# RozDavid/UnScene3D

Hardware: AMD Instinct MI355X
Metric: training scenes/sec (Res16UNet34C+Mask3D, 150k voxels) (higher is better)
Workload: dtype f32

## Files before the change

include/usc3d.h:

```cpp
#ifndef USC3D_H
#define USC3D_H

#include <stdint.h>

#ifdef __cplusplus
extern "C" {
#endif

typedef void* usc_stream_t;

enum usc_status {
  USC_OK = 0,
  USC_ERR_ARG = -1,
  USC_ERR_LAUNCH = -2,
  USC_ERR_RANGE = -3
};

const char* usc_last_error(void);
int usc_abi_version(void);
const char* usc_build_info(void);
int usc_device_count(void);


int usc_voxel_floor_f64(const double* xyz, int64_t n, double voxel_size,
// ... 65 lines not shown
                     usc_stream_t s);

int64_t usc_spconv_gather_gemm_ws_bytes(int64_t n_out, int32_t cin,
                                        int32_t cout, int32_t K);
int usc_spconv_gather_gemm(const float* in, int64_t n_in, int32_t cin,
                           const float* W, int32_t K, int32_t cout,
                           const int32_t* nbr, int64_t n_out,
                           const float* bias, float* out, int32_t accumulate, int32_t w_transposed,
                           void* ws, int64_t ws_bytes, usc_stream_t s);

int usc_spconv_pairs_gemm(const float* in, int32_t cin, const float* W,
                          int32_t K, int32_t cout, const int32_t* rows_in,
                          const int32_t* rows_out, const int64_t* koff,
                          int64_t P_capacity, float* out, usc_stream_t s);

int usc_cast_bf16(const float* in, int64_t n, uint16_t* out, usc_stream_t s);
int usc_spconv_pack_w_bf16(const float* W, int32_t K, int32_t cin, int32_t cout,
                           uint16_t* Wp, usc_stream_t s);
int64_t usc_spconv_gather_gemm_bf16_ws_bytes(int64_t n_out, int32_t cin,
                                             int32_t cout, int32_t K);
int usc_spconv_gather_gemm_bf16(const uint16_t* in, int64_t n_in, int32_t cin,
                                const uint16_t* Wp, int32_t K, int32_t cout,
                                const int32_t* nbr, int64_t n_out,
                                const float* bias, float* out, int32_t accumulate,
                                void* ws, int64_t ws_bytes, usc_stream_t s);

int64_t usc_spconv_wgrad_ws_bytes(int32_t K, int32_t cin, int32_t cout);
int usc_spconv_wgrad(const float* a, int32_t cin, const float* b, int32_t cout,
                     int32_t K, const int32_t* a_idx, const int32_t* b_idx,
                     const int64_t* koff, int64_t n_rows, float* dW, int32_t accumulate, void* ws,
                     int64_t ws_bytes, usc_stream_t s);
int64_t usc_spconv_wgrad_ws_bytes_rows(int32_t K, int32_t cin, int32_t cout,
                                       int64_t n_rows);
int64_t usc_spconv_wgrad_table_ws_bytes(int32_t K, int32_t cin, int32_t cout);
int usc_spconv_wgrad_table(const float* in, int32_t cin, const float* dy, int32_t cout, const int32_t* nbr, int32_t K,
                           int64_t n_out, float* dW, int32_t accumulate, void* ws, int64_t ws_bytes, usc_stream_t s);

void usc_spconv_wgrad_grid_limit(int32_t max_workgroups);
int32_t usc_spconv_wgrad_group_max(void);
int usc_spconv_wgrad_group_ok(int32_t R, int32_t cin, int32_t cout, int32_t K, int64_t n_rows);
int usc_spconv_wgrad_group(int32_t R, const float* const* a, const float* const* b, float* const* dW, int32_t cin,
                           int32_t cout, int32_t K, const int32_t* a_idx, const int32_t* b_idx, const int64_t* koff,
                           int64_t n_rows, int32_t accumulate, usc_stream_t s);

typedef struct usc_kmap {
  const int32_t* nbr;
  const int32_t* perm;
  const uint32_t* tile_mask;
  const int32_t* pair_in;
  const int32_t* pair_out;
  const int64_t* koff;
  int64_t n_in, n_out;
  int64_t pair_capacity;
  int32_t K;
  int32_t reserved;
} usc_kmap;

enum usc_conv_kind { USC_CONV_SAME = 0, USC_CONV_DOWN = 1, USC_CONV_UP = 2 };

typedef struct usc_bn {
  const float* gamma;
  const float* beta;
  float* running_mean;
  float* running_var;
  int64_t* num_batches_tracked;
  float eps, momentum;
// ... 398 lines not shown
```

unscene3d_amd/_lib.py:

```python
from __future__ import annotations

import ctypes as C
import os

import torch

_HERE = os.path.dirname(os.path.abspath(__file__))
LIB_PATH = os.environ.get("USC3D_LIB") or os.path.join(_HERE, "libusc3d_hip.so")

_p = C.c_void_p
_i32 = C.c_int32
_i64 = C.c_int64
_f64 = C.c_double
_f32 = C.c_float

class KMap(C.Structure):
    _fields_ = [("nbr", _p), ("perm", _p), ("tile_mask", _p), ("pair_in", _p), ("pair_out", _p), ("koff", _p),
                ("n_in", _i64), ("n_out", _i64), ("pair_capacity", _i64), ("K", _i32), ("reserved", _i32)]


class BNDesc(C.Structure):
    _fields_ = [("gamma", _p), ("beta", _p), ("running_mean", _p), ("running_var", _p), ("num_batches_tracked", _p),
                ("eps", _f32), ("momentum", _f32), ("c", _i32), ("training", _i32)]

# ... 26 lines not shown
    "usc_coordmap_capacity": (_i64, [_i64]),
    "usc_coordmap_ws_bytes": (_i64, [_i64]),
    "usc_coordmap_build": (C.c_int, [_p, _i64, _i32, _p, _p, _i64, _p, _p, _p, _p, _p, _i64, _p]),
    "usc_morton_cell_ids": (C.c_int, [_p, _i64, _i32, _i32, _i32, _i32, _i32, _p, _p]),
    "usc_kernel_map_cube": (C.c_int, [_p, _i64, _i32, _i32, _p, _p, _i64, _p, _p]),
    "usc_kernel_map_down2": (C.c_int, [_p, _i64, _i32, _p, _p, _i64, _p, _p, _p]),
    "usc_rulebook_ws_bytes": (_i64, [_i64, _i64]),
    "usc_rulebook_compact": (C.c_int, [_p, _i64, _i64, _p, _p, _p, _p, _i64, _p]),
    "usc_weight_transpose": (C.c_int, [_p, _i32, _i32, _i32, _i32, _p, _p]),
    "usc_spconv_plan": (C.c_int, [_i32, _i64, _i32, _i32, _i32]),
    "usc_spconv_gather_gemm_ws_bytes": (_i64, [_i64, _i32, _i32, _i32]),
    "usc_spconv_gather_gemm": (C.c_int, [_p, _i64, _i32, _p, _i32, _i32, _p, _i64, _p, _p, _i32, _i32, _p, _i64, _p]),
    "usc_rowsort_ws_bytes": (_i64, [_i32, _i64]),
    "usc_rowsort_build": (C.c_int, [_p, _i32, _i64, _p, _p, _p, _i64, _p]),
    "usc_spconv_sorted_ws_bytes": (_i64, [_i64, _i32, _i32, _i32]),
    "usc_spconv_sorted_gemm": (C.c_int, [_p, _i64, _i32, _p, _i32, _i32, _p, _p, _p, _i64, _p, _p, _i32, _i32, _p, _i64, _p]),
    "usc_spconv_sorted_gemm_ex": (C.c_int, [_p, _i64, _i32, _p, _i32, _i32, _p, _p, _p, _i64, _p, _p, _i32, _i32, _p, _i64, _p, _p]),
    "usc_group_reduce": (C.c_int, [_p, _i32, _i64, _i32, _p, _i32, _p, _p]),
    "usc_bn_tile_max_rows": (C.c_int64, []),
    "usc_bn_tile_ok": (C.c_int, [_i64, _i32]),
    "usc_bn_tile_ws_bytes": (C.c_int64, [_i32]),
    "usc_bn_tile_forward": (C.c_int, [_p, _i32, _p, _i64, _i32, _p, _p, _f32, _f32, _p, _p, _p, _p, _p, _p, _p, _p, _i32, _p,
                                      _p, _i64, _p]),
    "usc_bn_tile_backward": (C.c_int, [_p, _i32, _i32, _p, _p, _p, _p, _p, _p, _i64, _i32, _i32, _i32, _p, _p, _p, _p, _p,
                                       _i64, _p]),
    "usc_spconv_pairs_gemm": (C.c_int, [_p, _i32, _p, _i32, _i32, _p, _p, _p, _i64, _p, _p]),
    "usc_cast_bf16": (C.c_int, [_p, _i64, _p, _p]),
    "usc_spconv_pack_w_bf16": (C.c_int, [_p, _i32, _i32, _i32, _p, _p]),
    "usc_spconv_gather_gemm_bf16_ws_bytes": (_i64, [_i64, _i32, _i32, _i32]),
    "usc_spconv_gather_gemm_bf16": (C.c_int, [_p, _i64, _i32, _p, _i32, _i32, _p, _i64, _p, _p, _i32, _p, _i64, _p]),
    "usc_spconv_wgrad_ws_bytes": (_i64, [_i32, _i32, _i32]),
    "usc_spconv_wgrad": (C.c_int, [_p, _i32, _p, _i32, _i32, _p, _p, _p, _i64, _p, _i32, _p, _i64, _p]),
    "usc_spconv_wgrad_ws_bytes_rows": (_i64, [_i32, _i32, _i32, _i64]),
    "usc_step_size": (_i32, []),
    "usc_program_ws_bytes": (_i64, [_sp, _i32]),
    "usc_program_run": (C.c_int, [_sp, _i32, _i32, _p, _i64, _p]),
    "usc_spconv_wgrad_group_max": (_i32, []),
    "usc_spconv_wgrad_grid_limit": (None, [_i32]),
    "usc_spconv_wgrad_group_ok": (C.c_int, [_i32, _i32, _i32, _i32, _i64]),
    "usc_spconv_wgrad_group": (C.c_int, [_i32, _p, _p, _p, _i32, _i32, _i32, _p, _p, _p, _i64, _i32, _p]),
    "usc_spconv_wgrad_table_ws_bytes": (_i64, [_i32, _i32, _i32]),
    "usc_spconv_wgrad_table": (C.c_int, [_p, _i32, _p, _i32, _p, _i32, _i64, _p, _i32, _p, _i64, _p]),
    "usc_set_wgrad_lane": (C.c_int, [_p, _p, _i64, _i64]),
    "usc_wgrad_lane_join": (C.c_int, [_p]),
    "usc_wgrad_lane_hold": (C.c_int, [_i32, _i64, _i64, _p]),
    "usc_wgrad_lane_holding": (_i32, []),
    "usc_launch_stats_begin": (C.c_int, [_p, _i64, _p]),
    "usc_launch_stats_end": (_i64, [_p, _i64]),
    "usc_wall_clock_khz": (_i64, []),
    "usc_conv_ws_bytes": (_i64, [_kp, _i32, _i32, _i32]),
    "usc_unit_ws_bytes": (_i64, [_kp, _i32, _i32, _i32]),
    "usc_conv_forward": (C.c_int, [_kp, _i32, _p, _i32, _p, _i32, _p, _p, _p, _i64, _p]),
    "usc_conv_backward": (C.c_int, [_kp, _i32, _p, _i32, _p, _i32, _p, _p, _i32, _p, _i32, _p, _i64, _p]),
    "usc_bn_eval_stats": (C.c_int, [_p, _p, _p, _p, _f32, _i32, _p, _p, _p, _p, _p]),
    "usc_conv_bn_act_forward": (C.c_int, [_kp, _i32, _p, _i32, _p, _i32, _bp, _p, _i32, _p, _p, _p, _p, _i64, _p]),
    "usc_unit_bf16_ws_bytes": (_i64, [_kp, _i32, _i32, _i32]),
    "usc_conv_bn_act_forward_bf16": (C.c_int, [_kp, _i32, _p, _i32, _p, _i32, _bp, _p, _i32, _p, _p, _p, _p, _i64, _p]),
    "usc_conv_bn_act_backward": (C.c_int, [_kp, _i32, _p, _i32, _p, _i32, _bp, _p, _p, _p, _p, _p, _p, _p, _i32, _p,
                                           _i32, _p, _p, _i32, _p, _i64, _p]),
    "usc_colstats_ws_bytes": (_i64, [_i64, _i32]),
    "usc_colstats": (C.c_int, [_p, _p, _i64, _i32, _p, _p, _p, _i64, _p]),
    "usc_bn_apply": (C.c_int, [_p, _p, _p, _p, _i32, _p, _i64, _i32, _p]),
    "usc_bn_backward_dx": (C.c_int, [_p, _p, _p, _p, _p, _p, _p, _p, _p, _p, _i64, _i32, _p]),
    "usc_bn_backward_reduce": (C.c_int, [_p, _p, _p, _p, _p, _i64, _i32, _i32, _i32, _p, _p, _p, _p, _p, _i64, _p]),
    "usc_bn_forward_stats": (C.c_int, [_p, _i64, _i32, _p, _p, _f32, _f32, _p, _p, _p, _p, _p, _p, _p, _p, _i64, _p]),
    "usc_relu_fwd": (C.c_int, [_p, _p, _i64, _p]),
# ... 129 lines not shown
```

unscene3d_amd/csrc/units.hip:

```cpp
#include <stdlib.h>

#include <vector>

#include "common.h"

using namespace usc;

namespace {

struct WsCursor {
  char* base; int64_t bytes; int64_t off;
  void* take(int64_t n) {
    n = align_up(n > 0 ? n : 16, 256);
    if (off + n > bytes) return nullptr;
    void* p = base + off;
    off += n;
    return p;
  }
  int64_t left() const { return bytes - off; }
  void* rest() { return base + off; }
};

inline bool table_is_compact(int64_t n_out, int cin, int cout, int K) {
  return (usc_spconv_plan(0, n_out, cin, cout, K) >> 12) & 1;
// ... 24 lines not shown
    USC_REQUIRE(b == 0 || w, "usc unit: workspace too small (sorted gemm)");
    int32_t G = 0;
    const int rc = usc_spconv_sorted_gemm_ex(in, n_in, cin, W, K, cout, nbr, m->perm, m->tile_mask, n_out, bias, out,
                                             accumulate, wt, w, b, left ? &G : nullptr, s);
    if (!rc && left && G > 0) { left->partial = (const float*)w; left->G = G; }
    return rc;
  }
  if (wt && !compact) {
    float* Wt = (float*)ws.take((int64_t)K * cin * cout * 4);
    USC_REQUIRE(Wt, "usc unit: workspace too small (weight transpose)");
    int rc = usc_weight_transpose(W, K, cout, cin, K > 1 ? 1 : 0, Wt, s);
    if (rc) return rc;
    W = Wt;
    wt = 0;
  }
  const int64_t b = usc_spconv_gather_gemm_ws_bytes(n_out, cin, cout, K);
  void* w = b > 0 ? ws.take(b) : nullptr;
  USC_REQUIRE(b == 0 || w, "usc unit: workspace too small (gather gemm)");
  return usc_spconv_gather_gemm(in, n_in, cin, W, K, cout, nbr, n_out, bias, out, accumulate, wt, w, b, s);
}

struct HeldWgrad { const float* x; const float* dy; float* dW; const int32_t* a_idx; const int32_t* b_idx; const int64_t* koff;
                   int64_t rows, ws_bytes; int cin, cout, K; };
struct Lane { hipStream_t st = nullptr; hipEvent_t fork = nullptr, join = nullptr; void* ws = nullptr; int64_t ws_bytes = 0;
              int64_t max_rows = 0; bool dirty = false;
              bool hold = false; int64_t hold_min_rows = 0, release_max_rows = 0; std::vector<HeldWgrad> held; };
Lane g_lane[16];
Lane* lane_for_current_device() {
  int dev = 0;
  if (hipGetDevice(&dev) != hipSuccess || dev < 0 || dev >= 16) return nullptr;
  return g_lane[dev].st ? &g_lane[dev] : nullptr;
}

int lane_release(Lane* lane, usc_stream_t s) {
  lane->hold = false;
  if (lane->held.empty()) return USC_OK;
  if (hipEventRecord(lane->fork, as_stream(s)) != hipSuccess || hipStreamWaitEvent(lane->st, lane->fork, 0) != hipSuccess) {
    lane->held.clear();
    set_error("usc wgrad lane: releasing the held weight gradients failed (event)");
    return USC_ERR_LAUNCH;
  }
  int rc = USC_OK;
  lane->dirty = true;
  for (const HeldWgrad& h : lane->held) {
    rc = usc_spconv_wgrad(h.x, h.cin, h.dy, h.cout, h.K, h.a_idx, h.b_idx, h.koff, h.rows, h.dW, 1, lane->ws, h.ws_bytes,
                          (usc_stream_t)lane->st);
    if (rc) break;
  }
  lane->held.clear();
  return rc;
}

struct ConvShape { int64_t n_in, n_out; };
inline ConvShape conv_shape(const usc_kmap* m, int kind) {
  return kind == USC_CONV_UP ? ConvShape{m->n_out, m->n_in} : ConvShape{m->n_in, m->n_out};
}

int check_map(const usc_kmap* m, int kind, int cin, int cout, const char* who) {
  USC_REQUIRE(m, "%s: null kernel map", who);
  USC_REQUIRE(kind == USC_CONV_SAME || kind == USC_CONV_DOWN || kind == USC_CONV_UP, "%s: unknown conv kind %d", who, kind);
  USC_REQUIRE(cin >= 1 && cout >= 1 && m->K >= 1 && m->n_in >= 0 && m->n_out >= 0, "%s: bad sizes", who);
  USC_REQUIRE(m->nbr || (m->K == 1 && kind == USC_CONV_SAME), "%s: K>1 needs a neighbour table", who);
  USC_REQUIRE(kind != USC_CONV_SAME || m->n_in == m->n_out, "%s: a stride-1 map has n_in == n_out", who);
  return USC_OK;
}


__global__ __launch_bounds__(256) void cat_cols_kernel(const float4* __restrict__ a, int ca4, const float4* __restrict__ b,
                                                      int cb4, float4* __restrict__ dst, int64_t total4) {
  const int c4 = ca4 + cb4;
  for (int64_t e = (int64_t)blockIdx.x * 256 + threadIdx.x; e < total4; e += (int64_t)gridDim.x * 256) {
    const int64_t r = e / c4;
    const int j = (int)(e - r * c4);
    dst[e] = j < ca4 ? a[r * ca4 + j] : b[r * cb4 + (j - ca4)];
  }
}
__global__ __launch_bounds__(256) void split_cols_kernel(const float4* __restrict__ src, int ca4, int cb4, float4* __restrict__ da,
                                                        float4* __restrict__ db, int accumulate, int64_t total4) {
  const int c4 = ca4 + cb4;
// ... 102 lines not shown
int32_t usc_wgrad_lane_holding(void) {
  Lane* lane = lane_for_current_device();
  return lane && lane->hold ? 1 : 0;
}

int usc_wgrad_lane_join(usc_stream_t s) {
  Lane* lane = lane_for_current_device();
  if (lane && !lane->held.empty()) { const int rc = lane_release(lane, s); if (rc) return rc; }
  if (!lane || !lane->dirty) return USC_OK;
  if (hipEventRecord(lane->join, lane->st) != hipSuccess || hipStreamWaitEvent(as_stream(s), lane->join, 0) != hipSuccess) {
    set_error("usc_wgrad_lane_join: joining the lane failed");
    return USC_ERR_LAUNCH;
  }
  lane->dirty = false;
  return USC_OK;
}

static void conv_ws_parts(const usc_kmap* m, int kind, int cin, int cout, int64_t* fwd, int64_t* dgrad, int64_t* wg) {
  const int K = m->K;
  const ConvShape sh = conv_shape(m, kind);
  const int64_t wbytes = align_up((int64_t)K * cin * cout * 4, 256);
  if (kind == USC_CONV_SAME) {
    *fwd = table_gemm_ws(m, sh.n_out, cin, cout, K, false);
    *dgrad = table_gemm_ws(m, sh.n_in, cout, cin, K, true);
  } else if (kind == USC_CONV_DOWN) {
    *fwd = table_gemm_ws(m, sh.n_out, cin, cout, K, false);
    *dgrad = wbytes;
  } else {
    *fwd = 0;
    *dgrad = wbytes + table_gemm_ws(m, sh.n_in, cout, cin, K, false);
  }
  *dgrad = align_up(*dgrad + 256, 256);
  const int64_t rows = m->nbr ? m->pair_capacity : sh.n_in;
  *wg = align_up(usc_spconv_wgrad_ws_bytes_rows(K, cin, cout, rows), 256);
  if (kind == USC_CONV_SAME && m->nbr && cin <= 4 && cout == 32) {
    const int64_t t = align_up(usc_spconv_wgrad_table_ws_bytes(K, cin, cout), 256);
    if (t > *wg) *wg = t;
  }
}

int64_t usc_conv_ws_bytes(const usc_kmap* m, int32_t kind, int32_t cin, int32_t cout) {
  if (!m) return 0;
  int64_t fwd, dgrad, wg;
  conv_ws_parts(m, kind, cin, cout, &fwd, &dgrad, &wg);
  const int64_t bwd = dgrad + wg;
  return (fwd > bwd ? fwd : bwd) + 256;
}

static int conv_forward_impl(const usc_kmap* m, int32_t kind, const float* x, int32_t cin, const float* W, int32_t cout,
                             const float* bias, float* y, void* ws, int64_t ws_bytes, usc_stream_t s, Slices* left);

int usc_conv_forward(const usc_kmap* m, int32_t kind, const float* x, int32_t cin, const float* W, int32_t cout,
                     const float* bias, float* y, void* ws, int64_t ws_bytes, usc_stream_t s) {
  return conv_forward_impl(m, kind, x, cin, W, cout, bias, y, ws, ws_bytes, s, nullptr);
}

static int conv_forward_impl(const usc_kmap* m, int32_t kind, const float* x, int32_t cin, const float* W, int32_t cout,
                             const float* bias, float* y, void* ws, int64_t ws_bytes, usc_stream_t s, Slices* left) {
  if (left) *left = Slices{};
  int rc = check_map(m, kind, cin, cout, "usc_conv_forward");
  if (rc) return rc;
  const ConvShape sh = conv_shape(m, kind);
  if (sh.n_out == 0) return USC_OK;
  USC_REQUIRE(x && W && y, "usc_conv_forward: null pointer");
  WsCursor cur{(char*)ws, ws ? ws_bytes : 0, 0};
  if (kind == USC_CONV_UP) {
    USC_REQUIRE(m->pair_in && m->pair_out && m->koff, "usc_conv_forward: transposed conv needs the pair lists");
// ... 11 lines not shown
  p = Pending{};
  return rc;
}

static bool tile_form_on() {
  static const bool on = usc_bn_tile_max_rows() > 0;
  return on;
}
static bool tile_rows_ok(int64_t n, int c) { return tile_form_on() && n <= usc_bn_tile_max_rows() && usc_bn_tile_ok(n, c); }

static int conv_backward_impl(const usc_kmap* m, int32_t kind, const float* x, int32_t cin, const float* W, int32_t cout,
                              const float* dy, float* dx, int32_t dx_accumulate, float* dW, int32_t dW_accumulate, void* ws,
                              int64_t ws_bytes, usc_stream_t s, Pending* out);

int usc_conv_backward(const usc_kmap* m, int32_t kind, const float* x, int32_t cin, const float* W, int32_t cout,
                      const float* dy, float* dx, int32_t dx_accumulate, float* dW, int32_t dW_accumulate, void* ws,
                      int64_t ws_bytes, usc_stream_t s) {
  return conv_backward_impl(m, kind, x, cin, W, cout, dy, dx, dx_accumulate, dW, dW_accumulate, ws, ws_bytes, s, nullptr);
}

static int conv_backward_impl(const usc_kmap* m, int32_t kind, const float* x, int32_t cin, const float* W, int32_t cout,
                              const float* dy, float* dx, int32_t dx_accumulate, float* dW, int32_t dW_accumulate, void* ws,
                              int64_t ws_bytes, usc_stream_t s, Pending* out) {
  if (out) *out = Pending{};
  int rc = check_map(m, kind, cin, cout, "usc_conv_backward");
  if (rc) return rc;
  const ConvShape sh = conv_shape(m, kind);
  const int K = m->K;
  USC_REQUIRE(x && W && dy, "usc_conv_backward: null pointer");
  WsCursor cur{(char*)ws, ws ? ws_bytes : 0, 0};
  if (dW && dW_accumulate && x && dy) {
    Lane* lane = lane_for_current_device();
    const int64_t rows = m->nbr ? m->pair_capacity : sh.n_in;
    const int64_t b = usc_spconv_wgrad_ws_bytes_rows(K, cin, cout, rows);
    const bool lane_ok = lane && sh.n_in > 0 && sh.n_in <= lane->max_rows && sh.n_out <= lane->max_rows &&
                         b <= lane->ws_bytes && (!m->nbr || (m->pair_in && m->pair_out && m->koff));
    const int64_t big = sh.n_in > sh.n_out ? sh.n_in : sh.n_out;
    if (lane && lane->hold && big <= lane->release_max_rows) { rc = lane_release(lane, s); if (rc) return rc; }
    if (lane_ok && lane->hold && big >= lane->hold_min_rows) {
      HeldWgrad h{x, dy, dW, nullptr, nullptr, nullptr, m->nbr ? rows : sh.n_in, b, cin, cout, m->nbr ? K : 1};
      if (m->nbr) {
        h.a_idx = kind == USC_CONV_UP ? m->pair_out : m->pair_in;
        h.b_idx = kind == USC_CONV_UP ? m->pair_in : m->pair_out;
        h.koff = m->koff;
      }
      lane->held.push_back(h);
      dW = nullptr;
    } else if (lane_ok &&
        hipEventRecord(lane->fork, as_stream(s)) == hipSuccess && hipStreamWaitEvent(lane->st, lane->fork, 0) == hipSuccess) {
      usc_stream_t ls = (usc_stream_t)lane->st;
      lane->dirty = true;
      const int64_t bt = usc_spconv_wgrad_table_ws_bytes(K, cin, cout);
      if (kind == USC_CONV_SAME && m->nbr && cin <= 4 && cout == 32 && K <= 32 && bt <= lane->ws_bytes)
        rc = usc_spconv_wgrad_table(x, cin, dy, cout, m->nbr, K, sh.n_out, dW, 1, lane->ws, bt, ls);
      else if (!m->nbr)
        rc = usc_spconv_wgrad(x, cin, dy, cout, 1, nullptr, nullptr, nullptr, sh.n_in, dW, 1, lane->ws, b, ls);
      else if (kind == USC_CONV_UP)
        rc = usc_spconv_wgrad(x, cin, dy, cout, K, m->pair_out, m->pair_in, m->koff, rows, dW, 1, lane->ws, b, ls);
      else
        rc = usc_spconv_wgrad(x, cin, dy, cout, K, m->pair_in, m->pair_out, m->koff, rows, dW, 1, lane->ws, b, ls);
      if (rc) return rc;
      dW = nullptr;
    }
  }
  int64_t dgrad_bytes = 0;
  Slices left;
  const bool may_defer = out && dx && tile_rows_ok(sh.n_in, cin);
  if (may_defer) {
    int64_t f_, w_;
    conv_ws_parts(m, kind, cin, cout, &f_, &dgrad_bytes, &w_);
    if (dgrad_bytes + w_ > cur.bytes) dgrad_bytes = 0;
  }
  Slices* want = (may_defer && dgrad_bytes > 0) ? &left : nullptr;
  if (dx && sh.n_in > 0) {
    if (kind == USC_CONV_SAME) {
      rc = table_gemm(m, m->nbr, dy, sh.n_out, cout, W, K, cin, sh.n_in, nullptr, dx, dx_accumulate, 1, cur, s, want);
    } else if (kind == USC_CONV_DOWN) {
      USC_REQUIRE(!dx_accumulate, "usc_conv_backward: accumulate is not supported on the pair-list form");
      USC_REQUIRE(m->pair_in && m->pair_out && m->koff, "usc_conv_backward: strided conv needs the pair lists");
      float* Wt = (float*)cur.take((int64_t)K * cin * cout * 4);
      USC_REQUIRE(Wt, "usc_conv_backward: workspace too small");
      rc = usc_weight_transpose(W, K, cin, cout, 0, Wt, s);
      if (!rc) rc = usc_spconv_pairs_gemm(dy, cout, Wt, K, cin, m->pair_out, m->pair_in, m->koff, sh.n_in, dx, s);
    } else {
      float* Wt = (float*)cur.take((int64_t)K * cin * cout * 4);
      USC_REQUIRE(Wt, "usc_conv_backward: workspace too small");
      rc = usc_weight_transpose(W, K, cin, cout, 0, Wt, s);
      if (!rc) rc = table_gemm(m, m->nbr, dy, sh.n_out, cout, Wt, K, cin, sh.n_in, nullptr, dx, dx_accumulate, 0, cur, s, want);
    }
    if (!rc && left.G > 0) {
      out->dx = dx; out->partial = left.partial; out->G = left.G; out->n = sh.n_in; out->c = cin; out->accumulate = dx_accumulate;
    }
    if (rc) dW = nullptr;
  }
  if (dW) {
    WsCursor wc{(char*)ws, ws ? ws_bytes : 0, left.G > 0 ? dgrad_bytes : 0};
    const int64_t rows = m->nbr ? m->pair_capacity : sh.n_in;
    const int64_t b = usc_spconv_wgrad_ws_bytes_rows(K, cin, cout, rows);
    void* w = wc.take(b);
    if (!w) set_error("usc_conv_backward: workspace too small (weight gradient)");
    const int64_t bt = usc_spconv_wgrad_table_ws_bytes(K, cin, cout);
    if (!w) rc = USC_ERR_ARG;
    else if (kind == USC_CONV_SAME && m->nbr && cin <= 4 && cout == 32 && K <= 32 && (char*)w + bt <= (char*)ws + ws_bytes)
      rc = usc_spconv_wgrad_table(x, cin, dy, cout, m->nbr, K, sh.n_out, dW, dW_accumulate, w, bt, s);
    else if (!m->nbr)
      rc = usc_spconv_wgrad(x, cin, dy, cout, 1, nullptr, nullptr, nullptr, sh.n_in, dW, dW_accumulate, w, b, s);
    else if (kind == USC_CONV_UP)
      rc = usc_spconv_wgrad(x, cin, dy, cout, K, m->pair_out, m->pair_in, m->koff, rows, dW, dW_accumulate, w, b, s);
    else
      rc = usc_spconv_wgrad(x, cin, dy, cout, K, m->pair_in, m->pair_out, m->koff, rows, dW, dW_accumulate, w, b, s);
  }
  return rc;
}

int64_t usc_unit_ws_bytes(const usc_kmap* m, int32_t kind, int32_t cin, int32_t cout) {
  return usc_conv_ws_bytes(m, kind, cin, cout) + align_up(usc_colstats_ws_bytes(0, cout), 256) +
         align_up(2 * (int64_t)cout * 4, 256) + 256;
}

int usc_conv_bn_act_forward(const usc_kmap* m, int32_t kind, const float* x, int32_t cin, const float* W, int32_t cout,
                            const usc_bn* bn, const float* residual, int32_t relu, float* y, float* stats, float* out,
                            void* ws, int64_t ws_bytes, usc_stream_t s) {
  USC_REQUIRE(bn && bn->c == cout, "usc_conv_bn_act_forward: batch-norm width must equal the conv's output width");
  USC_REQUIRE(y && stats && out && bn->gamma && bn->beta, "usc_conv_bn_act_forward: null pointer");
  const ConvShape sh = conv_shape(m, kind);
  WsCursor cur{(char*)ws, ws ? ws_bytes : 0, 0};
  const int64_t sb = usc_colstats_ws_bytes(sh.n_out, cout);
  void* sws = cur.take(sb);
  USC_REQUIRE(sws, "usc_conv_bn_act_forward: workspace too small");
  const bool tile = bn->training && tile_rows_ok(sh.n_out, cout) && sb >= usc_bn_tile_ws_bytes(cout);
  Slices left;
  int rc = conv_forward_impl(m, kind, x, cin, W, cout, nullptr, y, cur.rest(), cur.left(), s, tile ? &left : nullptr);
  if (rc) return rc;
  if (sh.n_out == 0) return USC_OK;
  float* mean = stats, *invstd = stats + cout, *scale = stats + 2 * cout, *shift = stats + 3 * cout;
  if (tile)
    return usc_bn_tile_forward(left.partial, left.G, y, sh.n_out, cout, bn->gamma, bn->beta, bn->eps, bn->momentum,
                               bn->running_mean, bn->running_var, bn->num_batches_tracked, mean, invstd, scale, shift,
                               residual, relu, out, sws, sb, s);
// ... 224 lines not shown
```

unscene3d_amd/ops.py:

```python
from __future__ import annotations

from dataclasses import dataclass

import ctypes
import os

import torch

from . import profiler as _prof
from ._lib import check, lib, require_device


def _stream():
    return torch._C._cuda_getCurrentRawStream(torch._C._cuda_getDevice())


def _chk(t: torch.Tensor, dtype, name: str):
    if not isinstance(t, torch.Tensor):
        raise RuntimeError(f"{name} must be a torch.Tensor")
    if not t.is_cuda:
        raise RuntimeError(f"{name} must be a HIP (cuda) tensor — unscene3d_amd has no CPU path")
    if t.dtype != dtype:
        raise RuntimeError(f"{name} must be {dtype}, got {t.dtype}")
    if not t.is_contiguous():
# ... 326 lines not shown


PARAMS_FINAL_HOOK = None


def _params_final(params):
    if PARAMS_FINAL_HOOK is not None and params:
        PARAMS_FINAL_HOOK(params)


def _grad_written(*params):
    _join_after_backward()
    if GRAD_WRITTEN_HOOK is not None:
        for p in params:
            if p is not None:
                GRAD_WRITTEN_HOOK(p)


def wgrad(a, b, K, a_idx=None, b_idx=None, koff=None, into=None, out=None, nbr=None):
    _chk(a, torch.float32, "a")
    _chk(b, torch.float32, "b")
    cin, cout = a.shape[1], b.shape[1]
    dW = into if into is not None else (out if out is not None else
                                        torch.empty((K, cin, cout), dtype=torch.float32, device=a.device))
    if nbr is not None and cin <= 4 and cout == 32 and K <= 32 and nbr.shape == (K, b.shape[0]):
        wsb = lib.usc_spconv_wgrad_table_ws_bytes(K, cin, cout)
        ws = _ws(wsb, a.device)
        with _prof.maybe(lambda: "usc::stem_wgrad_kernel" + (f" [n={b.shape[0]} cin={cin} cout={cout} K={K}]" if _prof.SHAPES else ""),
                         lambda: _conv_cost(_prof.table_pairs(nbr), a.shape[0], b.shape[0], K, cin, cout)):
            check(lib.usc_spconv_wgrad_table(_ptr(a), cin, _ptr(b), cout, _ptr(nbr), K, b.shape[0], _ptr(dW),
                                             int(into is not None), _ptr(ws), ws.numel(), _stream()),
                  "usc_spconv_wgrad_table")
        return dW
    ws = _ws(lib.usc_spconv_wgrad_ws_bytes(K, cin, cout), a.device)
    n_rows = a.shape[0] if a_idx is None else int(a_idx.shape[0])
    with _prof.maybe(lambda: _kernel_symbol(2, n_rows, cin, cout, K),
                     lambda: _conv_cost(n_rows if koff is None else int(koff[-1].item()), a.shape[0], b.shape[0], K,
                                        cin, cout)):
        check(lib.usc_spconv_wgrad(_ptr(a), cin, _ptr(b), cout, K, _ptr(a_idx), _ptr(b_idx), _ptr(koff), n_rows,
                                   _ptr(dW), int(into is not None), _ptr(ws), ws.numel(), _stream()), "usc_spconv_wgrad")
    return dW


def wgrad_group(a_list, b_list, into_list, K, a_idx, b_idx, koff):
    import ctypes as C
    R = len(a_list)
    if not (R == len(b_list) == len(into_list) and 1 <= R <= lib.usc_spconv_wgrad_group_max()):
        raise RuntimeError("wgrad_group: between 1 and usc_spconv_wgrad_group_max() problems, three lists of equal length")
    cin, cout = a_list[0].shape[1], b_list[0].shape[1]
    for a, b, w in zip(a_list, b_list, into_list):
        _chk(a, torch.float32, "a")
        _chk(b, torch.float32, "b")
        _chk(w, torch.float32, "dW")
        if a.shape[1] != cin or b.shape[1] != cout or w.numel() != K * cin * cout:
            raise RuntimeError("wgrad_group: the problems of a group have one shape")
    n_rows = a_list[0].shape[0] if a_idx is None else int(a_idx.shape[0])
    pa = (C.c_void_p * R)(*[t.data_ptr() for t in a_list])
    pb = (C.c_void_p * R)(*[t.data_ptr() for t in b_list])
    pw = (C.c_void_p * R)(*[t.data_ptr() for t in into_list])
    check(lib.usc_spconv_wgrad_group(R, pa, pb, pw, cin, cout, K, _ptr(a_idx), _ptr(b_idx), _ptr(koff), n_rows, 1,
                                     _stream()), "usc_spconv_wgrad_group")
    return into_list


class _ConvSame(torch.autograd.Function):

    @staticmethod
    def forward(ctx, feats, W, bias, nbr, get_rulebook):
        feats = feats.contiguous()
        W3 = W if W.dim() == 3 else W[None]
        out = gather_gemm(feats, W3.contiguous(), nbr, feats.shape[0], bias=None if bias is None else bias.reshape(-1))
        ctx.save_for_backward(feats, W3)
        ctx.nbr, ctx.get_rulebook = nbr, get_rulebook
# ... 632 lines not shown


def _lin_bwd(dy2, x2, W, dW_out, db_out, need_dx=True, accumulate=False, add=None, y_relu=None, dx_add=None,
             dx_add2=None, want_dx_b=False):
    M, N = dy2.shape
    K = x2.shape[1]
    if want_dx_b or dx_add2 is not None:
        if not need_dx:
            return (None, None) if want_dx_b else None
        if _small_linear_ok(M, K, N):
            dx = torch.empty((M, K), dtype=torch.float32, device=dy2.device)
            dx_b = torch.empty_like(dx) if want_dx_b else None
            check(lib.usc_linear_bwd_ex2(_ptr(dy2), _ptr(y_relu), _ptr(x2), _ptr(add), _ptr(W), M, N, K, _ptr(dx),
                                         _ptr(dx_add), _ptr(dx_add2), _ptr(dx_b), _ptr(dW_out), _ptr(db_out),
                                         int(accumulate), _stream()), "usc_linear_bwd")
        else:
            dx_b = _lin_bwd(dy2, x2, W, dW_out, db_out, True, accumulate, add, y_relu, dx_add)
            dx = dx_b if dx_add2 is None else dx_b + dx_add2
        return (dx, dx_b) if want_dx_b else dx
    if _small_linear_ok(M, K, N):
        dx = torch.empty((M, K), dtype=torch.float32, device=dy2.device) if need_dx else None
        check(lib.usc_linear_bwd_ex(_ptr(dy2), _ptr(y_relu), _ptr(x2), _ptr(add), _ptr(W), M, N, K, _ptr(dx),
                                    _ptr(dx_add) if need_dx else None, _ptr(dW_out), _ptr(db_out), int(accumulate),
                                    _stream()), "usc_linear_bwd")
        return dx
    if y_relu is not None:
        dy2 = dy2 * (y_relu > 0)
    if add is not None:
        x2 = x2 + add
    if dx_add is not None:
        dx = _lin_bwd(dy2, x2, W, dW_out, db_out, need_dx, accumulate)
        return None if dx is None else dx.add_(dx_add)
    rows_ok = _rows_gemm_ok(M, K, N) and W.is_contiguous()
    if rows_ok and dW_out.is_contiguous():
        if accumulate:
            wgrad(dy2, x2, 1, into=dW_out)
        else:
            wgrad(dy2, x2, 1, out=dW_out)
    elif accumulate:
        dW_out.addmm_(dy2.t(), x2)
    else:
        torch.mm(dy2.t(), x2, out=dW_out)
    if db_out is not None:
        col_sum(dy2, db_out, accumulate)
    if not need_dx:
        return None
    if rows_ok:
        return gather_gemm(dy2, W.view(1, N, K), None, M)
    return dy2 @ W


class _LinearRows(torch.autograd.Function):
    @staticmethod
    def forward(ctx, x, W, b, relu=False, passthrough=False, pad_rows_to=None):
        x2 = x.contiguous().view(-1, x.shape[-1])
        ctx.rows = x2.shape[0]
        if pad_rows_to is not None:
            if relu or passthrough or x2.shape[0] != x.shape[-2] or pad_rows_to < x2.shape[0]:
                raise RuntimeError("linear: pad_rows_to is for one [.., M, K] table, M <= pad_rows_to, without relu")
            y = _lin_fwd(x2, W, b, pad_rows_to=pad_rows_to)
            ctx.save_for_backward(x2, W, None)
            ctx.has_bias, ctx.shape = b is not None, x.shape
            ctx.w_param, ctx.b_param = W, b
            return y.view(*x.shape[:-2], int(pad_rows_to), W.shape[0])
        y = _lin_fwd(x2, W, b, relu=relu)
        ctx.save_for_backward(x2, W, y if relu else None)
        ctx.has_bias, ctx.shape = b is not None, x.shape
        ctx.w_param, ctx.b_param = W, b
        y = y.view(*x.shape[:-1], W.shape[0])
        return (y, x) if passthrough else y

    @staticmethod
    def backward(ctx, dy, dres=None):
        x2, W, y_relu = ctx.saved_tensors
        dy2 = dy.contiguous().view(-1, W.shape[0])[:ctx.rows]
        tw = _grad_target(ctx.w_param)
# ... 322 lines not shown
```

Measured before the change: 43.84.

## Add MFMA split-M dense weight-gradient kernel for identity 1x1 convs and linears

After: 43.81. No clear change (-0.1%).

```diff
diff --git a/include/usc3d.h b/include/usc3d.h
--- a/include/usc3d.h
+++ b/include/usc3d.h
@@ -121,6 +121,11 @@
                      int64_t ws_bytes, usc_stream_t s);
 int64_t usc_spconv_wgrad_ws_bytes_rows(int32_t K, int32_t cin, int32_t cout,
                                        int64_t n_rows);
+int32_t usc_dense_wgrad_ok(int64_t M, int32_t Ca, int32_t Cb);
+int64_t usc_dense_wgrad_ws_bytes(int64_t M, int32_t Ca, int32_t Cb, int32_t with_bias);
+int usc_dense_wgrad(const float* A, int32_t Ca, const float* B, int32_t Cb, int64_t M, float* dW, float* dbias,
+                    int32_t accumulate, void* ws, int64_t ws_bytes, usc_stream_t s);
+void usc_dense_wgrad_grid_limit(int32_t max_workgroups);
 int64_t usc_spconv_wgrad_table_ws_bytes(int32_t K, int32_t cin, int32_t cout);
 int usc_spconv_wgrad_table(const float* in, int32_t cin, const float* dy, int32_t cout, const int32_t* nbr, int32_t K,
                            int64_t n_out, float* dW, int32_t accumulate, void* ws, int64_t ws_bytes, usc_stream_t s);
diff --git a/unscene3d_amd/_lib.py b/unscene3d_amd/_lib.py
--- a/unscene3d_amd/_lib.py
+++ b/unscene3d_amd/_lib.py
@@ -82,6 +82,10 @@
     "usc_spconv_wgrad_ws_bytes": (_i64, [_i32, _i32, _i32]),
     "usc_spconv_wgrad": (C.c_int, [_p, _i32, _p, _i32, _i32, _p, _p, _p, _i64, _p, _i32, _p, _i64, _p]),
     "usc_spconv_wgrad_ws_bytes_rows": (_i64, [_i32, _i32, _i32, _i64]),
+    "usc_dense_wgrad_ok": (_i32, [_i64, _i32, _i32]),
+    "usc_dense_wgrad_ws_bytes": (_i64, [_i64, _i32, _i32, _i32]),
+    "usc_dense_wgrad": (C.c_int, [_p, _i32, _p, _i32, _i64, _p, _p, _i32, _p, _i64, _p]),
+    "usc_dense_wgrad_grid_limit": (None, [_i32]),
     "usc_step_size": (_i32, []),
     "usc_program_ws_bytes": (_i64, [_sp, _i32]),
     "usc_program_run": (C.c_int, [_sp, _i32, _i32, _p, _i64, _p]),
diff --git a/unscene3d_amd/csrc/dense_wgrad.hip b/unscene3d_amd/csrc/dense_wgrad.hip
--- /dev/null
+++ b/unscene3d_amd/csrc/dense_wgrad.hip
@@ -0,0 +1,244 @@
+#include "common.h"
+
+namespace usc {
+
+typedef float dw_f32x16 __attribute__((ext_vector_type(16)));
+
+struct DenseWgradParams {
+  const float* A;
+  const float* B;
+  int64_t M, L;
+  int Ca, Cb;
+  int S, btiles, tiles, items;
+  float* partial;
+  float* bpartial;
+  float* dW;
+  float* dbias;
+  int accumulate;
+};
+
+template <int NB>
+__global__ __launch_bounds__(256) void dense_wgrad_kernel(DenseWgradParams p) {
+  __shared__ float red[4][NB * 16][64];
+  __shared__ float bred[4][32];
+  const int lane = threadIdx.x & 63, wave = threadIdx.x >> 6;
+  const int i = lane & 31, h = lane >> 5;
+  const int Ca = p.Ca, Cb = p.Cb;
+  for (int item = blockIdx.x; item < p.items; item += gridDim.x) {
+    const int s = item / p.tiles, t = item - s * p.tiles;
+    const int at = t / p.btiles, bt = t - at * p.btiles;
+    const int ca0 = at * 32, cb0 = bt * 32 * NB;
+    const bool bias_wg = p.dbias != nullptr && bt == 0;
+    int64_t rb = ((int64_t)s * 4 + wave) * p.L;
+    if (rb > p.M) rb = p.M;
+    int64_t re = rb + p.L;
+    if (re > p.M) re = p.M;
+
+    dw_f32x16 acc[NB];
+#pragma unroll
+    for (int nb = 0; nb < NB; ++nb)
+#pragma unroll
+      for (int r = 0; r < 16; ++r) acc[nb][r] = 0.f;
+    float bsum = 0.f;
+
+    const float* ap = p.A + ca0 + i;
+    const float* bp = p.B + cb0 + NB * i;
+    auto load = [&](int64_t q, float (&av)[8], float (&bv)[8][NB]) __attribute__((always_inline)) {
+#pragma unroll
+      for (int u = 0; u < 8; ++u) {
+        const int64_t row = q + 2 * u + h;
+        av[u] = ap[row * Ca];
+        if (NB == 2) {
+          const float2 v = *reinterpret_cast<const float2*>(bp + row * Cb);
+          bv[u][0] = v.x; bv[u][1 % NB] = v.y;
+        } else {
+          bv[u][0] = bp[row * Cb];
+        }
+      }
+    };
+    auto run = [&](const float (&av)[8], const float (&bv)[8][NB]) __attribute__((always_inline)) {
+#pragma unroll
+      for (int u = 0; u < 8; ++u)
+#pragma unroll
+        for (int nb = 0; nb < NB; ++nb)
+          acc[nb] = __builtin_amdgcn_mfma_f32_32x32x2f32(av[u], bv[u][nb], acc[nb], 0, 0, 0);
+      if (bias_wg) {
+#pragma unroll
+        for (int u = 0; u < 8; ++u) bsum += av[u];
+      }
+    };
+    const int64_t nfull = (re - rb) >> 4;
+    float aX[8], aY[8], bX[8][NB], bY[8][NB];
+    if (nfull > 0) {
+      load(rb, aX, bX);
+      for (int64_t b = 0; b < nfull; b += 2) {
+        const int64_t b1 = b + 1 < nfull ? b + 1 : nfull - 1, b2 = b + 2 < nfull ? b + 2 : nfull - 1;
+        load(rb + b1 * 16, aY, bY);
+        run(aX, bX);
+        load(rb + b2 * 16, aX, bX);
+        if (b + 1 < nfull) run(aY, bY);
+      }
+    }
+    const int64_t qt = rb + nfull * 16;
+    if (qt < re) {
+#pragma unroll
+      for (int u = 0; u < 8; ++u) {
+        const int64_t row = qt + 2 * u + h;
+        const bool ok = row < re;
+        aY[u] = ok ? ap[row * Ca] : 0.f;
+#pragma unroll
+        for (int nb = 0; nb < NB; ++nb) bY[u][nb] = ok ? bp[row * Cb + nb] : 0.f;
+      }
+      run(aY, bY);
+    }
+
+#pragma unroll
+    for (int nb = 0; nb < NB; ++nb)
+#pragma unroll
+      for (int r = 0; r < 16; ++r) red[wave][nb * 16 + r][lane] = acc[nb][r];
+    if (bias_wg) {
+      const float other = __shfl(bsum, i + 32, 64);
+      if (h == 0) bred[wave][i] = bsum + other;
+    }
+    __syncthreads();
+    const bool direct = p.S == 1;
+    const bool rmw = direct && p.accumulate;
+    float* dst = direct ? p.dW : p.partial + (int64_t)s * Ca * Cb;
+    const bool vec_ok = NB == 2 && (reinterpret_cast<uintptr_t>(dst) & 7) == 0;
+#pragma unroll
+    for (int rr = 0; rr < 4; ++rr) {
+      const int r = 4 * wave + rr;
+      float v[NB];
+#pragma unroll
+      for (int nb = 0; nb < NB; ++nb) {
+        float tsum = red[0][nb * 16 + r][lane] + red[1][nb * 16 + r][lane];
+        tsum += red[2][nb * 16 + r][lane];
+        tsum += red[3][nb * 16 + r][lane];
+        v[nb] = tsum;
+      }
+      const int ca = ca0 + (r & 3) + 8 * (r >> 2) + 4 * h;
+      float* o = dst + (int64_t)ca * Cb + cb0 + NB * i;
+      if (vec_ok) {
+        float2 w2 = make_float2(v[0], v[1 % NB]);
+        if (rmw) {
+          const float2 old = *reinterpret_cast<const float2*>(o);
+          w2.x += old.x; w2.y += old.y;
+        }
+        *reinterpret_cast<float2*>(o) = w2;
+      } else {
+#pragma unroll
+        for (int nb = 0; nb < NB; ++nb) o[nb] = rmw ? o[nb] + v[nb] : v[nb];
+      }
+    }
+    if (bias_wg && wave == 0 && h == 0) {
+      float v = bred[0][i] + bred[1][i];
+      v += bred[2][i];
+      v += bred[3][i];
+      float* o = (direct ? p.dbias : p.bpartial + (int64_t)s * Ca) + ca0 + i;
+      *o = rmw ? *o + v : v;
+    }
+    __syncthreads();
+  }
+}
+
+__global__ __launch_bounds__(256) void dense_wgrad_reduce_kernel(const float* __restrict__ partial,
+                                                                const float* __restrict__ bpartial, int S, int64_t numel,
+                                                                int nbias, int accumulate, float* __restrict__ dW,
+                                                                float* __restrict__ dbias) {
+  const int64_t total = numel + nbias;
+  for (int64_t j = (int64_t)blockIdx.x * 256 + threadIdx.x; j < total; j += (int64_t)gridDim.x * 256) {
+    const bool w = j < numel;
+    const float* src = w ? partial + j : bpartial + (j - numel);
+    const int64_t stride = w ? numel : nbias;
+    float* out = w ? dW + j : dbias + (j - numel);
+    float v = 0.f;
+    int s = 0;
+    for (; s + 16 <= S; s += 16) {
+      float t[16];
+#pragma unroll
+      for (int u = 0; u < 16; ++u) t[u] = src[(int64_t)(s + u) * stride];
+#pragma unroll
+      for (int u = 0; u < 16; ++u) v += t[u];
+    }
+    for (; s < S; ++s) v += src[(int64_t)s * stride];
+    *out = accumulate ? *out + v : v;
+  }
+}
+
+namespace {
+struct DensePlan { int NB, btiles, tiles, S; int64_t L; };
+
+DensePlan dense_plan(int64_t M, int Ca, int Cb) {
+  DensePlan pl;
+  pl.NB = (Cb % 64 == 0) ? 2 : 1;
+  pl.btiles = Cb / (32 * pl.NB);
+  pl.tiles = (Ca / 32) * pl.btiles;
+  const int64_t target = M >= 65536 ? 1024 : 512;
+  int64_t S = target / pl.tiles;
+  const int64_t by_rows = M / 64 + 1;
+  if (S > by_rows) S = by_rows;
+  const int64_t by_bytes = M * (Ca + Cb) / (2 * (int64_t)Ca * Cb);
+  if (S > by_bytes) S = by_bytes;
+  if (S > 128) S = 128;
+  if (S < 1) S = 1;
+  int64_t L = align_up(ceil_div(M > 0 ? M : 1, 4 * S), 16);
+  S = ceil_div(M > 0 ? M : 1, 4 * L);
+  pl.S = (int)S;
+  pl.L = L;
+  return pl;
+}
+bool dense_shape_ok(int64_t M, int Ca, int Cb) {
+  return M >= 0 && Ca >= 32 && Cb >= 32 && Ca % 32 == 0 && Cb % 32 == 0 && Ca <= 4096 && Cb <= 4096;
+}
+int g_dense_grid_limit = 0;
+}
+}
+
+extern "C" {
+
+void usc_dense_wgrad_grid_limit(int32_t max_workgroups) { usc::g_dense_grid_limit = max_workgroups; }
+
+int32_t usc_dense_wgrad_ok(int64_t M, int32_t Ca, int32_t Cb) { return usc::dense_shape_ok(M, Ca, Cb) ? 1 : 0; }
+
+int64_t usc_dense_wgrad_ws_bytes(int64_t M, int32_t Ca, int32_t Cb, int32_t with_bias) {
+  if (!usc::dense_shape_ok(M, Ca, Cb) || M == 0) return 0;
+  const usc::DensePlan pl = usc::dense_plan(M, Ca, Cb);
+  if (pl.S == 1) return 0;
+  return (int64_t)pl.S * ((int64_t)Ca * Cb + (with_bias ? Ca : 0)) * 4;
+}
+
+int usc_dense_wgrad(const float* A, int32_t Ca, const float* B, int32_t Cb, int64_t M, float* dW, float* dbias,
+                    int32_t accumulate, void* ws, int64_t ws_bytes, usc_stream_t s) {
+  USC_REQUIRE(usc::dense_shape_ok(M, Ca, Cb),
+              "usc_dense_wgrad: channel counts must be multiples of 32 in [32, 4096] and M >= 0 (got %d, %d, %lld)", Ca, Cb,
+              (long long)M);
+  USC_REQUIRE(dW, "usc_dense_wgrad: null pointer");
+  if (M == 0) return USC_OK;
+  USC_REQUIRE(A && B, "usc_dense_wgrad: null pointer");
+  const usc::DensePlan pl = usc::dense_plan(M, Ca, Cb);
+  USC_REQUIRE(pl.NB == 1 || (reinterpret_cast<uintptr_t>(B) & 7) == 0, "usc_dense_wgrad: B must be 8-byte aligned");
+  const int64_t numel = (int64_t)Ca * Cb;
+  const int64_t need = usc_dense_wgrad_ws_bytes(M, Ca, Cb, dbias != nullptr);
+  USC_REQUIRE(need == 0 || (ws && ws_bytes >= need), "usc_dense_wgrad: workspace too small");
+  USC_REQUIRE(need == 0 || (reinterpret_cast<uintptr_t>(ws) & 15) == 0, "usc_dense_wgrad: workspace must be 16-byte aligned");
+  hipStream_t st = usc::as_stream(s);
+  usc::DenseWgradParams p{};
+  p.A = A; p.B = B; p.M = M; p.L = pl.L; p.Ca = Ca; p.Cb = Cb;
+  p.S = pl.S; p.btiles = pl.btiles; p.tiles = pl.tiles; p.items = pl.S * pl.tiles;
+  p.partial = (float*)ws;
+  p.bpartial = (float*)ws + (int64_t)pl.S * numel;
+  p.dW = dW; p.dbias = dbias; p.accumulate = accumulate;
+  int grid = p.items;
+  if (usc::g_dense_grid_limit > 0 && grid > usc::g_dense_grid_limit) grid = usc::g_dense_grid_limit;
+  if (pl.NB == 2) hipLaunchKernelGGL(usc::dense_wgrad_kernel<2>, dim3((unsigned)grid), dim3(256), 0, st, p);
+  else hipLaunchKernelGGL(usc::dense_wgrad_kernel<1>, dim3((unsigned)grid), dim3(256), 0, st, p);
+  if (pl.S > 1) {
+    const int nbias = dbias ? Ca : 0;
+    hipLaunchKernelGGL(usc::dense_wgrad_reduce_kernel, dim3((unsigned)usc::stream_grid(numel + nbias, 256)), dim3(256), 0, st,
+                       (const float*)p.partial, (const float*)p.bpartial, pl.S, numel, nbias, (int)accumulate, dW, dbias);
+  }
+  USC_CHECK_LAUNCH("usc_dense_wgrad");
+  return USC_OK;
+}
+
+}
diff --git a/unscene3d_amd/csrc/units.hip b/unscene3d_amd/csrc/units.hip
--- a/unscene3d_amd/csrc/units.hip
+++ b/unscene3d_amd/csrc/units.hip
@@ -80,6 +80,20 @@
   return g_lane[dev].st ? &g_lane[dev] : nullptr;
 }
 
+inline bool dense_wgrad_case(bool identity, int K, int cin, int cout, int64_t rows) {
+  return identity && K == 1 && rows > 0 && usc_dense_wgrad_ok(rows, cin, cout);
+}
+inline int64_t wgrad_ws_need(bool identity, int K, int cin, int cout, int64_t rows) {
+  return dense_wgrad_case(identity, K, cin, cout, rows) ? usc_dense_wgrad_ws_bytes(rows, cin, cout, 0)
+                                                        : usc_spconv_wgrad_ws_bytes_rows(K, cin, cout, rows);
+}
+inline int wgrad_identity(const float* x, int cin, const float* dy, int cout, int64_t rows, float* dW, int accumulate, void* ws,
+                          int64_t ws_bytes, usc_stream_t s) {
+  if (dense_wgrad_case(true, 1, cin, cout, rows))
+    return usc_dense_wgrad(x, cin, dy, cout, rows, dW, nullptr, accumulate, ws, ws_bytes, s);
+  return usc_spconv_wgrad(x, cin, dy, cout, 1, nullptr, nullptr, nullptr, rows, dW, accumulate, ws, ws_bytes, s);
+}
+
 int lane_release(Lane* lane, usc_stream_t s) {
   lane->hold = false;
   if (lane->held.empty()) return USC_OK;
@@ -91,8 +105,11 @@
   int rc = USC_OK;
   lane->dirty = true;
   for (const HeldWgrad& h : lane->held) {
-    rc = usc_spconv_wgrad(h.x, h.cin, h.dy, h.cout, h.K, h.a_idx, h.b_idx, h.koff, h.rows, h.dW, 1, lane->ws, h.ws_bytes,
-                          (usc_stream_t)lane->st);
+    if (!h.a_idx)
+      rc = wgrad_identity(h.x, h.cin, h.dy, h.cout, h.rows, h.dW, 1, lane->ws, h.ws_bytes, (usc_stream_t)lane->st);
+    else
+      rc = usc_spconv_wgrad(h.x, h.cin, h.dy, h.cout, h.K, h.a_idx, h.b_idx, h.koff, h.rows, h.dW, 1, lane->ws, h.ws_bytes,
+                            (usc_stream_t)lane->st);
     if (rc) break;
   }
   lane->held.clear();
@@ -261,7 +278,7 @@
   }
   *dgrad = align_up(*dgrad + 256, 256);
   const int64_t rows = m->nbr ? m->pair_capacity : sh.n_in;
-  *wg = align_up(usc_spconv_wgrad_ws_bytes_rows(K, cin, cout, rows), 256);
+  *wg = align_up(wgrad_ws_need(!m->nbr, K, cin, cout, rows), 256);
   if (kind == USC_CONV_SAME && m->nbr && cin <= 4 && cout == 32) {
     const int64_t t = align_up(usc_spconv_wgrad_table_ws_bytes(K, cin, cout), 256);
     if (t > *wg) *wg = t;
@@ -339,7 +356,7 @@
   if (dW && dW_accumulate && x && dy) {
     Lane* lane = lane_for_current_device();
     const int64_t rows = m->nbr ? m->pair_capacity : sh.n_in;
-    const int64_t b = usc_spconv_wgrad_ws_bytes_rows(K, cin, cout, rows);
+    const int64_t b = wgrad_ws_need(!m->nbr, K, cin, cout, rows);
     const bool lane_ok = lane && sh.n_in > 0 && sh.n_in <= lane->max_rows && sh.n_out <= lane->max_rows &&
                          b <= lane->ws_bytes && (!m->nbr || (m->pair_in && m->pair_out && m->koff));
     const int64_t big = sh.n_in > sh.n_out ? sh.n_in : sh.n_out;
@@ -361,7 +378,7 @@
       if (kind == USC_CONV_SAME && m->nbr && cin <= 4 && cout == 32 && K <= 32 && bt <= lane->ws_bytes)
         rc = usc_spconv_wgrad_table(x, cin, dy, cout, m->nbr, K, sh.n_out, dW, 1, lane->ws, bt, ls);
       else if (!m->nbr)
-        rc = usc_spconv_wgrad(x, cin, dy, cout, 1, nullptr, nullptr, nullptr, sh.n_in, dW, 1, lane->ws, b, ls);
+        rc = wgrad_identity(x, cin, dy, cout, sh.n_in, dW, 1, lane->ws, b, ls);
       else if (kind == USC_CONV_UP)
         rc = usc_spconv_wgrad(x, cin, dy, cout, K, m->pair_out, m->pair_in, m->koff, rows, dW, 1, lane->ws, b, ls);
       else
@@ -403,7 +420,7 @@
   if (dW) {
     WsCursor wc{(char*)ws, ws ? ws_bytes : 0, left.G > 0 ? dgrad_bytes : 0};
     const int64_t rows = m->nbr ? m->pair_capacity : sh.n_in;
-    const int64_t b = usc_spconv_wgrad_ws_bytes_rows(K, cin, cout, rows);
+    const int64_t b = wgrad_ws_need(!m->nbr, K, cin, cout, rows);
     void* w = wc.take(b);
     if (!w) set_error("usc_conv_backward: workspace too small (weight gradient)");
     const int64_t bt = usc_spconv_wgrad_table_ws_bytes(K, cin, cout);
@@ -411,7 +428,7 @@
     else if (kind == USC_CONV_SAME && m->nbr && cin <= 4 && cout == 32 && K <= 32 && (char*)w + bt <= (char*)ws + ws_bytes)
       rc = usc_spconv_wgrad_table(x, cin, dy, cout, m->nbr, K, sh.n_out, dW, dW_accumulate, w, bt, s);
     else if (!m->nbr)
-      rc = usc_spconv_wgrad(x, cin, dy, cout, 1, nullptr, nullptr, nullptr, sh.n_in, dW, dW_accumulate, w, b, s);
+      rc = wgrad_identity(x, cin, dy, cout, sh.n_in, dW, dW_accumulate, w, b, s);
     else if (kind == USC_CONV_UP)
       rc = usc_spconv_wgrad(x, cin, dy, cout, K, m->pair_out, m->pair_in, m->koff, rows, dW, dW_accumulate, w, b, s);
     else
diff --git a/unscene3d_amd/ops.py b/unscene3d_amd/ops.py
--- a/unscene3d_amd/ops.py
+++ b/unscene3d_amd/ops.py
@@ -382,13 +382,34 @@
                                              int(into is not None), _ptr(ws), ws.numel(), _stream()),
                   "usc_spconv_wgrad_table")
         return dW
+    n_rows = a.shape[0] if a_idx is None else int(a_idx.shape[0])
+    if a_idx is None and K == 1 and n_rows > 0 and lib.usc_dense_wgrad_ok(n_rows, cin, cout):
+        return dense_wgrad(a, b, dW, None, into is not None)
     ws = _ws(lib.usc_spconv_wgrad_ws_bytes(K, cin, cout), a.device)
-    n_rows = a.shape[0] if a_idx is None else int(a_idx.shape[0])
     with _prof.maybe(lambda: _kernel_symbol(2, n_rows, cin, cout, K),
                      lambda: _conv_cost(n_rows if koff is None else int(koff[-1].item()), a.shape[0], b.shape[0], K,
                                         cin, cout)):
         check(lib.usc_spconv_wgrad(_ptr(a), cin, _ptr(b), cout, K, _ptr(a_idx), _ptr(b_idx), _ptr(koff), n_rows,
                                    _ptr(dW), int(into is not None), _ptr(ws), ws.numel(), _stream()), "usc_spconv_wgrad")
+    return dW
+
+
+def dense_wgrad(a, b, dW, db=None, accumulate=False):
+    _chk(a, torch.float32, "a")
+    _chk(b, torch.float32, "b")
+    M, Ca = a.shape
+    Cb = b.shape[1]
+    if b.shape[0] != M or not dW.is_contiguous() or dW.dtype != torch.float32 or dW.numel() != Ca * Cb:
+        raise RuntimeError("dense_wgrad: a [M, Ca], b [M, Cb] and a contiguous f32 dW of Ca*Cb elements")
+    if db is not None and (not db.is_contiguous() or db.dtype != torch.float32 or db.numel() != Ca):
+        raise RuntimeError("dense_wgrad: `db` must be a contiguous f32 vector with one entry per column of a")
+    wsb = lib.usc_dense_wgrad_ws_bytes(M, Ca, Cb, int(db is not None))
+    ws = _ws(max(wsb, 16), a.device)
+    with _prof.maybe(lambda: f"usc::dense_wgrad_kernel<{2 if Cb % 64 == 0 else 1}>" +
+                     (f" [n={M} cin={Ca} cout={Cb} K=1]" if _prof.SHAPES else ""),
+                     lambda: _conv_cost(M, M, M, 1, Ca, Cb)):
+        check(lib.usc_dense_wgrad(_ptr(a), Ca, _ptr(b), Cb, M, _ptr(dW), _ptr(db), int(accumulate), _ptr(ws), wsb,
+                                  _stream()), "usc_dense_wgrad")
     return dW
 
 
@@ -1087,16 +1108,15 @@
         dx = _lin_bwd(dy2, x2, W, dW_out, db_out, need_dx, accumulate)
         return None if dx is None else dx.add_(dx_add)
     rows_ok = _rows_gemm_ok(M, K, N) and W.is_contiguous()
+    db_done = False
     if rows_ok and dW_out.is_contiguous():
-        if accumulate:
-            wgrad(dy2, x2, 1, into=dW_out)
-        else:
-            wgrad(dy2, x2, 1, out=dW_out)
+        db_done = db_out is not None and db_out.is_contiguous()
+        dense_wgrad(dy2, x2, dW_out, db_out if db_done else None, accumulate)
     elif accumulate:
         dW_out.addmm_(dy2.t(), x2)
     else:
         torch.mm(dy2.t(), x2, out=dW_out)
-    if db_out is not None:
+    if db_out is not None and not db_done:
         col_sum(dy2, db_out, accumulate)
     if not need_dx:
         return None
```
